# jrkerns/pylinac

Measured on NVIDIA H100. Metric: EPID frames/sec (1024x1024) through PicketFence.analyze(), higher is better.
Workload: dtype u16 pixels / int exact sums / f64 profiles

## Files before the change

pylinac_b200/csrc/common.cuh:

```cuda
#pragma once
#include <cuda_runtime.h>
#include <cstdint>
#include <cstdio>
#include <cstring>
#include <string>
#include <unordered_map>
#include <vector>

#include "../../include/epid.h"

namespace epid {

void set_error(const char* fmt, ...);

#define EPID_CUDA(call)                                                                      \
    do {                                                                                     \
        cudaError_t _e = (call);                                                             \
        if (_e != cudaSuccess) {                                                             \
            ::epid::set_error("%s failed: %s (%s:%d)", #call, cudaGetErrorString(_e), __FILE__, __LINE__); \
            return EPID_ERR_CUDA;                                                            \
        }                                                                                    \
    } while (0)

#define EPID_REQUIRE(cond, code, ...)              \
// ... 19 lines not shown
struct epid_ctx {
    int device = 0;
    int sm_count = 0;
    int cc_major = 0, cc_minor = 0;
    size_t hbm_bytes = 0;
    cudaStream_t stream = nullptr;
    cudaStream_t copy_stream[2] = {nullptr, nullptr};
    int64_t launches = 0;
    void* nccl_comm = nullptr;
    int nranks = 1, rank = 0;
    void* scratch = nullptr;
    size_t scratch_bytes = 0;
    void* scratch2 = nullptr;
    size_t scratch2_bytes = 0;
    void* hist_scratch = nullptr;
    size_t hist_bytes = 0;
    void* inv_scratch = nullptr;
    size_t inv_bytes = 0;
    int stats_exact = 0;
    int64_t stats_uncertified = 0;
    void* pinned = nullptr;
    size_t pinned_bytes = 0;
    void* pinned_ring = nullptr;
    size_t pinned_ring_bytes = 0;
    int pf_exact_only = 0;
    int pf_win2 = 1;
    int64_t pf_fallbacks = 0;
    int64_t pf_redone_frames = 0;
    int64_t pf_exact_frames = 0;
    cudaStream_t redo_stream = nullptr;
    cudaEvent_t ev_front = nullptr, ev_main_done = nullptr, ev_redo_done = nullptr;
    int* h_flags = nullptr;
    std::unordered_map<const void*, size_t> smem_optin;
};

constexpr size_t EPID_BATCH_PAD = 256;
struct epid_batch {
    epid_ctx* ctx = nullptr;
    int dtype = EPID_U16;
    int n = 0, h = 0, w = 0;
    void* dptr = nullptr;
    void* base = nullptr;
    bool owns = true;
    size_t bytes() const { return (size_t)n * h * w * epid::dtype_size(dtype); }
};

namespace epid {
int ensure_scratch(epid_ctx* ctx, size_t bytes);
int ensure_pinned(epid_ctx* ctx, size_t bytes);

template <class K>
inline int smem_opt_in(epid_ctx* ctx, K* kernel, size_t bytes) {
    size_t& cur = ctx->smem_optin[(const void*)kernel];
    if (bytes > cur) {
        EPID_CUDA(cudaFuncSetAttribute(kernel, cudaFuncAttributeMaxDynamicSharedMemorySize, (int)bytes));
        cur = bytes;
    }
    return EPID_OK;
}
#define EPID_SMEM_OPT_IN(ctx, kernel, bytes) do { int _rc = ::epid::smem_opt_in(ctx, kernel, bytes); if (_rc != EPID_OK) return _rc; } while (0)

#ifdef __CUDACC__
__device__ __forceinline__ uint4 ldg_stream16(const void* p) {
    uint4 r;
    asm volatile("ld.global.nc.L1::no_allocate.v4.u32 {%0,%1,%2,%3}, [%4];"
                 : "=r"(r.x), "=r"(r.y), "=r"(r.z), "=r"(r.w)
                 : "l"(p));
    return r;
}

template <typename T>
__device__ __forceinline__ T warp_sum(T v) {
#pragma unroll
    for (int o = 16; o > 0; o >>= 1) v += __shfl_xor_sync(0xffffffffu, v, o);
    return v;
}
template <typename T>
__device__ __forceinline__ T warp_min(T v) {
#pragma unroll
    for (int o = 16; o > 0; o >>= 1) v = min(v, __shfl_xor_sync(0xffffffffu, v, o));
    return v;
}
template <typename T>
__device__ __forceinline__ T warp_max(T v) {
#pragma unroll
    for (int o = 16; o > 0; o >>= 1) v = max(v, __shfl_xor_sync(0xffffffffu, v, o));
    return v;
}
#endif

}
```

pylinac_b200/csrc/pf.cu:

```cuda
#include <cmath>
#include <condition_variable>
#include <cstdlib>
#include <mutex>
#include <thread>
#include <pthread.h>
#include <sched.h>

#define EPID_PK_MAXBLK 2
#include "pf_common.cuh"

namespace epid {

__global__ void k_pf_init(const uint16_t* base, int n, int H0, int W0, int crop, FrameRef* refs, PfFrame* fr, int* counters, const int* __restrict__ sel) {
    const int i = blockIdx.x * blockDim.x + threadIdx.x;
    if (i == 0) { counters[0] = 0; counters[1] = 0; counters[2] = 0; }
    if (i >= n) return;
    refs[i].origin = base + (size_t)(sel ? sel[i] : i) * H0 * W0 + (size_t)crop * W0 + crop;
    refs[i].pitch = W0;
    refs[i].pad = 0;
    PfFrame& f = fr[i];
    f.status = EPID_PF_OK;
    f.noisy = 0;
    f.inv = 0;
    f.corner_inverted = 0;
// ... 83 lines not shown
                            csum[k] += cl;
                            rs += cl;
                        }
                    }
                    rs = warp_sum(rs);
                    if (lane == 0) atomicAdd(&rowsum_sm[rr], rs);
                }
            }
        }
#pragma unroll
        for (int k = 0; k < 8; k++) colpart[tid * 8 + k] = active ? csum[k] : 0u;
        __syncthreads();
        for (int x = tid; x < g.W; x += STATS_THREADS) {
            const int ac = x + mis;
            uint32_t s = 0;
            for (int gg = 0; gg < g.groups; gg++) s += colpart[(gg * g.vprp) * 8 + ac];
            colsum2[(size_t)fi * g.W + x] = s;
        }
        for (int y = tid; y < g.H; y += STATS_THREADS) rowsum2[(size_t)fi * g.H + y] = rowsum_sm[y];
        __syncthreads();
    }
}

__global__ void __launch_bounds__(PROF_THREADS)
k_pf_profile(const PfConst* __restrict__ cc, PfFrame* fr, const uint32_t* __restrict__ rowsum, const uint32_t* __restrict__ colsum,
             const uint32_t* __restrict__ rowsum2, const uint32_t* __restrict__ colsum2) {
    extern __shared__ __align__(16) unsigned char smraw[];
    const int fi = blockIdx.x;
    const PfConst& c = *cc;
    pf_profile_block(c, fr[fi], rowsum + (size_t)fi * c.H, colsum + (size_t)fi * c.W, rowsum2 + (size_t)fi * c.H,
                     colsum2 + (size_t)fi * c.W, smraw);
}

__global__ void __launch_bounds__(WIN_WARPS * 32)
k_pf_windows(const PfConst* __restrict__ cc, const FrameRef* __restrict__ frames, PfFrame* fr, PfWin* __restrict__ wins, int todo_only) {
    __shared__ __align__(16) uint16_t s_px[WIN_WARPS][WIN_CAP_PX];
    __shared__ uint32_t s_m2[WIN_WARPS][WIN_MAX_NC];
    const int fi = blockIdx.y;
    const PfConst& c = *cc;
    PfFrame& f = fr[fi];
    if (f.status != EPID_PF_OK) return;
    if (todo_only && !f.todo) return;
    const int wid = threadIdx.x >> 5, lane = threadIdx.x & 31;
    for (int li = blockIdx.x; li < f.n_inview; li += gridDim.x) {
    const int H = c.H, W = c.W;
    const int orient = f.orientation;
    const int leaf = f.inview[li];
    const double dpmm = c.p.dpmm;
    const double lw_px = c.p.leaf_width_mm[leaf] * dpmm;
    const double lc_px = c.p.leaf_center_mm[leaf] * dpmm + (orient == 0 ? (double)H / 2.0 : (double)W / 2.0);
    const FrameRef frf = frames[fi];
    const int inv = f.inv;
    const uint32_t mn = f.mn, mx = f.mx;
    const double Dd = (double)f.D;
    uint16_t* px = s_px[wid];
    uint32_t* m2 = s_m2[wid];
    double* xs = reinterpret_cast<double*>(px);

    for (int pk = wid; pk < f.n_pickets; pk += WIN_WARPS) {
        PfWin& out = wins[((size_t)fi * PF_L + li) * PF_P + pk];
        if (todo_only && out.valid != -1) continue;
        const double pidx = (double)f.picket_idx[pk];
        const double spacing = f.spacing;
        int a0 = max((int)(pidx - spacing / 2.0), 0);
        int a1 = min((int)(pidx + spacing / 2.0), orient == 0 ? W : H);
        int b0 = max((int)(lc_px - lw_px / 2.0), 0);
        int b1 = min((int)(lc_px + lw_px / 2.0), orient == 0 ? H : W);
        const int nc = a1 - a0, nr = b1 - b0;
        if (nc <= 0 || nr <= 0) {
            if (lane == 0) { out.valid = 0; out.l = 0; out.r = 0; f.status = EPID_PF_WINDOW_NO_PEAK; }
            continue;
        }
        if (nc > WIN_MAX_NC || nr > WIN_MAX_NR) {
            if (lane == 0) { out.valid = 0; f.status = EPID_PF_CAPACITY; }
            continue;
        }
        const int cw = min(nc, WIN_CAP_PX / nr);
        const int sag = c.p.sag_px;
        const int k1 = (nr - 1) / 2, k2 = nr / 2;
        uint32_t gmax = 0;
        unsigned long long rs1[2] = {0, 0}, rs2[2] = {0, 0};
        uint32_t lmin = 0xffffffffu, lmax = 0;
        for (int j0 = 0; j0 < nc; j0 += cw) {
            const int cn = min(cw, nc - j0);
            __syncwarp();
            if (orient == 0) {
                for (int t = lane; t < nr * cn; t += 32) {
                    const int i = t / cn, jj = t - i * cn;
                    int row = b0 + i - sag;
                    row %= H; if (row < 0) row += H;
                    const uint32_t v = __ldg(frf.origin + (size_t)row * frf.pitch + a0 + j0 + jj);
                    const uint32_t g = inv ? mx - v : v - mn;
                    px[i * cn + jj] = (uint16_t)g;
                    gmax = max(gmax, g);
// ... 114 lines not shown
            }
        }
#pragma unroll
        for (int o = 16; o > 0; o >>= 1) {
            const double op = __shfl_xor_sync(0xffffffffu, best_prom, o);
            const int oi = __shfl_xor_sync(0xffffffffu, best_idx, o);
            const int olb = __shfl_xor_sync(0xffffffffu, best_lb, o);
            const int orb = __shfl_xor_sync(0xffffffffu, best_rb, o);
            if (op > best_prom || (op == best_prom && oi > best_idx)) { best_prom = op; best_idx = oi; best_lb = olb; best_rb = orb; }
        }
        if (best_idx < 0) {
            if (lane == 0) { out.valid = 0; f.status = EPID_PF_WINDOW_NO_PEAK; }
            __syncwarp();
            continue;
        }
        if (lane == 0) {
            const int p = best_idx;
            const double h = xs[p] - best_prom * 0.5;
            int k = p;
            while (best_lb < k && h < xs[k]) k--;
            double l = (double)k;
            if (xs[k] < h) l += (h - xs[k]) / (xs[k + 1] - xs[k]);
            k = p;
            while (k < best_rb && h < xs[k]) k++;
            double r = (double)k;
            if (xs[k] < h) r -= (h - xs[k]) / (xs[k - 1] - xs[k]);
            out.valid = 1;
            out.l = l;
            out.r = r;
        }
        __syncwarp();
    }
    }
}

struct PfWork {
    FrameRef* refs;
    FrameRef* refs_b;
    ValueMap* maps;
    PfFrame* fr;
    FrameStats* stats;
    uint32_t *rowsum, *colsum, *rowsum2, *colsum2;
    PfWin* wins;
    epid_pf_summary* summ;
    epid_pf_meas* meas;
    PfConst* cst;
    int* counters;
    int* select;
    int* sel_idx;
    void* front;
    PfWinRec* winrec;
    size_t total;
};

static size_t align_up(size_t v, size_t a) { return (v + a - 1) / a * a; }

static void carve(PfWork& w, char* base, int n, int H, int W, int meas_cap) {
    size_t o = 0;
    auto take = [&](size_t bytes) { char* p = base ? base + o : nullptr; o = align_up(o + bytes, 256); return p; };
    w.refs = (FrameRef*)take(sizeof(FrameRef) * n);
    w.refs_b = (FrameRef*)take(sizeof(FrameRef) * n);
    w.maps = (ValueMap*)take(sizeof(ValueMap) * n);
    w.fr = (PfFrame*)take(sizeof(PfFrame) * n);
    w.stats = (FrameStats*)take(sizeof(FrameStats) * n);
    w.rowsum = (uint32_t*)take(sizeof(uint32_t) * (size_t)n * H);
    w.colsum = (uint32_t*)take(sizeof(uint32_t) * (size_t)n * W);
// ... 236 lines not shown
        ctx->launches++;
        hc.post_filter = 1;
        EPID_CUDA(cudaMemcpyAsync(w.cst, &hc, sizeof(hc), cudaMemcpyHostToDevice, stream));
        StatsGeom g2 = g;
        g2.box = 0;
        rc = launch_frame_stats(ctx, stream, g2, w.refs, n, w.stats, w.rowsum, w.colsum);
        if (rc != EPID_OK) return rc;
        k_pf_decide<<<nb, tb, 0, stream>>>(w.cst, w.stats, w.fr, n, nullptr, 0, w.counters);
        ctx->launches++;
    }
    if (p->orientation < 0) {
        const size_t smem = sizeof(uint32_t) * (size_t)(STATS_THREADS * 8 + H);
        EPID_SMEM_OPT_IN(ctx, k_pf_clamp_sums, 64 * 1024);
        const int grid = n < ctx->sm_count ? n : ctx->sm_count;
        k_pf_clamp_sums<<<grid, STATS_THREADS, smem, stream>>>(g, w.refs, w.fr, n, w.rowsum2, w.colsum2);
        ctx->launches++;
    }
    {
        const size_t smem = pf_profile_smem_bytes(PROF_THREADS, H, W);
        EPID_SMEM_OPT_IN(ctx, k_pf_profile, smem);
        k_pf_profile<<<n, PROF_THREADS, smem, stream>>>(w.cst, w.fr, w.rowsum, w.colsum, w.rowsum2, w.colsum2);
        ctx->launches++;
    }
    if (tm) { rc = tm->mark(stream, PF_STAGE_EXACT_FRONT); if (rc != EPID_OK) return rc; }
    }
    {
        if (hc.win2) {
            rc = launch_pf_windows2(ctx, stream, w.cst, w.refs, w.fr, w.winrec, w.wins, n, tm);
            if (rc != EPID_OK) return rc;
        }
        rc = launch_pf_windows_fast(ctx, stream, w.cst, w.refs, w.fr, w.wins, n);
        if (rc != EPID_OK) return rc;
        if (tm) { rc = tm->mark(stream, PF_STAGE_WINDOWS); if (rc != EPID_OK) return rc; }
        dim3 grid(p->n_leaves < 8 ? p->n_leaves : 8, n);
        k_pf_windows<<<grid, WIN_WARPS * 32, 0, stream>>>(w.cst, w.refs, w.fr, w.wins, 1);
        ctx->launches++;
        if (tm) { rc = tm->mark(stream, PF_STAGE_WINDOWS_GENERIC); if (rc != EPID_OK) return rc; }
    }
    rc = launch_pf_finalize(ctx, stream, w.cst, w.fr, w.wins, w.summ, w.meas, n, meas_cap);
    if (rc != EPID_OK) return rc;
    if (tm) { rc = tm->mark(stream, PF_STAGE_FINALIZE); if (rc != EPID_OK) return rc; }
    EPID_CUDA(cudaGetLastError());
    return EPID_OK;
}

static int ensure_scratch2(epid_ctx* ctx, size_t bytes) {
    if (ctx->scratch2_bytes >= bytes) return EPID_OK;
    if (ctx->scratch2) { EPID_CUDA(cudaStreamSynchronize(ctx->stream)); EPID_CUDA(cudaFree(ctx->scratch2)); ctx->scratch2 = nullptr; ctx->scratch2_bytes = 0; }
    cudaError_t e = cudaMalloc(&ctx->scratch2, bytes);
    if (e != cudaSuccess) { set_error("cudaMalloc(%zu) failed: %s", bytes, cudaGetErrorString(e)); return EPID_ERR_NOMEM; }
    ctx->scratch2_bytes = bytes;
    return EPID_OK;
}

static bool pf_fast_ok(const epid_ctx* ctx, const epid_pf_params* p, int H0, int W0) {
    const int H = H0 - 2 * p->crop_px, W = W0 - 2 * p->crop_px;
    return !ctx->pf_exact_only && p->filter_size == 0 && pf_front_supported(H, W, W0);
}


static int pf_redo_deferred(epid_ctx* ctx, cudaStream_t stream, const uint16_t* d_frames, int m, int H0, int W0, const epid_pf_params* p,
                            int meas_cap, PfWork& w, uint16_t** pools, cudaEvent_t after = nullptr) {
    const int H = H0 - 2 * p->crop_px, W = W0 - 2 * p->crop_px;
    const int Wp = (W + 7) / 8 * 8;
    const int chunk = m < PF_REDO_CHUNK ? m : PF_REDO_CHUNK;
    PfWork rw;
    carve(rw, nullptr, chunk, H, W, meas_cap);
    const size_t work_bytes = align_up(rw.total, 256);
// ... 414 lines not shown
```

pylinac_b200/csrc/pf_common.cuh:

```cuda
#pragma once
#include <cmath>

#include "filters.cuh"
#include "peaks.cuh"
#include "stats.cuh"

namespace epid {

constexpr int PF_P = EPID_PF_MAX_PICKETS;
constexpr int PF_L = EPID_PF_MAX_LEAVES;
constexpr int PROF_THREADS = 256;
constexpr int PROF_MAXN = STATS_MAX_DIM;
constexpr int PROF_PEAK_CAP = 512;
constexpr int WIN_WARPS = 4;
constexpr int WIN_CAP_PX = 4096;
constexpr int WIN_MAX_NC = 1024;
constexpr int WIN_MAX_NR = 64;
constexpr int FIN_THREADS = 256;

constexpr int PF_STATUS_DEFERRED = 90;

struct PfConst {
    epid_pf_params p;
    int H, W;
// ... 7 lines not shown
struct PfFrame {
    int status;
    int noisy;
    int inv;
    int corner_inverted;
    int noise_passes;
    uint32_t mn, mx, D;
    uint32_t med2;
    int orientation;
    int n_pickets;
    int n_inview;
    int todo;
    int win2;
    int picket_idx[PF_P];
    double picket_val[PF_P];
    double spacing;
    short inview[PF_L];
};

struct PfWin { int valid; double l, r; };

constexpr int PF_W2_NCW = 64;
constexpr int PF_W2_NRW = 32;
constexpr int PF_W2_WCAP = 1024;
constexpr int PF_W2_POOL = PF_W2_WCAP * PF_W2_NCW;
struct alignas(16) PfWinRec {
    uint32_t hdr;
    uint32_t moff;
    uint32_t pad[2];
    unsigned long long num[PF_W2_NRW];
    uint32_t ext[PF_W2_NRW];
};
static_assert(sizeof(PfWinRec) == 400, "PfWinRec layout");

__device__ inline void pf_decide_frame(const PfConst& c, const FrameStats& s, PfFrame& f, int check_noise, int* counters) {
    f.mn = s.mn;
    f.mx = s.mx;
    f.D = s.mx - s.mn;
    if (f.D == 0) { f.status = EPID_PF_FLAT_IMAGE; f.noisy = 0; return; }
    if (!c.post_filter) {
        if (check_noise) {
            const double near_min = np_lerp((double)s.ostat[0], (double)s.ostat[1], c.lo.gamma);
            const double near_max = np_lerp((double)s.ostat[2], (double)s.ostat[3], c.hi.gamma);
            const double mnv = (double)s.mn, mxv = (double)s.mx;
            const bool max_is_extreme = mxv > near_max * 1.25;
            const bool min_is_extreme = (mnv < near_min * 0.75) && (fabs(mnv - near_min) > 0.1 * (near_max - near_min));
            f.noisy = (max_is_extreme || min_is_extreme) ? 1 : 0;
            if (f.noisy) atomicAdd(&counters[0], 1);
        }
        const double avg = (double)s.corner_sum / (double)(4 * 10 * 10);
        const double mean = (double)s.sum / (double)s.npix;
        f.corner_inverted = avg > mean ? 1 : 0;
    }
    const int inv = (c.post_filter ? 0 : f.corner_inverted) ^ (c.p.invert ? 1 : 0);
    f.inv = inv;
    const uint32_t a = s.ostat[4], b = s.ostat[5];
    f.med2 = inv ? (s.mx - b) + (s.mx - a) : (a - s.mn) + (b - s.mn);
}


struct PfTimers {
    std::vector<cudaEvent_t> ev;
    bool on = false;
    int record(cudaStream_t s) {
        cudaEvent_t e;
        EPID_CUDA(cudaEventCreate(&e));
// ... 280 lines not shown
```

pylinac_b200/csrc/pf_win_common.cuh:

```cuda
#pragma once
#include <utility>

#include "pf_common.cuh"

namespace epid {

__device__ __forceinline__ unsigned long long mad_wide_u32(uint32_t a, uint32_t b, unsigned long long c) {
    unsigned long long d;
    asm("mad.wide.u32 %0, %1, %2, %3;" : "=l"(d) : "r"(a), "r"(b), "l"(c));
    return d;
}

struct NetList {
    int n;
    short a[640], b[640];
};
constexpr NetList batcher_net(int N) {
    NetList L{};
    for (int p = 1; p < N; p <<= 1)
        for (int k = p; k >= 1; k >>= 1)
            for (int j = k % p; j <= N - 1 - k; j += 2 * k)
                for (int i = 0; i < k; i++)
                    if (i <= N - j - k - 1 && (i + j) / (2 * p) == (i + j + k) / (2 * p)) {
                        L.a[L.n] = (short)(i + j);
                        L.b[L.n] = (short)(i + j + k);
                        L.n++;
                    }
    return L;
}
template <int N>
struct BatcherNet {
    static constexpr NetList L = batcher_net(N);
};

template <int A, int B, int N>
__device__ __forceinline__ void cmpswap_u16x2(uint32_t (&r)[N]) {
    const uint32_t a = r[A], b = r[B];
    r[A] = __vminu2(a, b);
    r[B] = __vmaxu2(a, b);
}
template <int N, int... I>
__device__ __forceinline__ void apply_net_u16x2(uint32_t (&r)[N], std::integer_sequence<int, I...>) {
    (cmpswap_u16x2<BatcherNet<N>::L.a[I], BatcherNet<N>::L.b[I], N>(r), ...);
}
template <int N>
__device__ __forceinline__ void sort_net_u16x2(uint32_t (&r)[N]) {
    apply_net_u16x2<N>(r, std::make_integer_sequence<int, BatcherNet<N>::L.n>{});
}

template <int A, int B, int N>
__device__ __forceinline__ void cmpswap_u64(unsigned long long (&r)[N]) {
    const unsigned long long a = r[A], b = r[B];
    r[A] = a < b ? a : b;
    r[B] = a < b ? b : a;
}
template <int N, int... I>
__device__ __forceinline__ void apply_net_u64(unsigned long long (&r)[N], std::integer_sequence<int, I...>) {
    (cmpswap_u64<BatcherNet<N>::L.a[I], BatcherNet<N>::L.b[I], N>(r), ...);
}
template <int A, int B, int N>
__device__ __forceinline__ void cmpswap_f64(double (&r)[N]) {
    const double a = r[A], b = r[B];
    r[A] = fmin(a, b);
    r[B] = fmax(a, b);
}
template <int N, int... I>
__device__ __forceinline__ void apply_net_f64(double (&r)[N], std::integer_sequence<int, I...>) {
    (cmpswap_f64<BatcherNet<N>::L.a[I], BatcherNet<N>::L.b[I], N>(r), ...);
}
template <int N>
__device__ __forceinline__ void sort_net_f64(double (&r)[N]) {
    apply_net_f64<N>(r, std::make_integer_sequence<int, BatcherNet<N>::L.n>{});
}

template <int N>
__device__ __forceinline__ void sort_net_u64(unsigned long long (&r)[N]) {
    apply_net_u64<N>(r, std::make_integer_sequence<int, BatcherNet<N>::L.n>{});
}

template <int N>
__device__ __forceinline__ void pair_median_exact(const uint16_t* __restrict__ px, int S, int t, uint32_t& m_lo, uint32_t& m_hi) {
    uint32_t r[N];
#pragma unroll
    for (int i = 0; i < N; i++) r[i] = *reinterpret_cast<const uint32_t*>(px + i * S + 2 * t);
    sort_net_u16x2<N>(r);
    const uint32_t va = r[(N - 1) / 2], vb = r[N / 2];
    m_lo = (va & 0xffffu) + (vb & 0xffffu);
    m_hi = (va >> 16) + (vb >> 16);
}

template <int NRP>
__device__ __forceinline__ void pair_median_padded(const uint16_t* __restrict__ px, int S, int nr, int t, uint32_t& m_lo, uint32_t& m_hi) {
    uint32_t r[NRP];
#pragma unroll
    for (int i = 0; i < NRP; i++)
        r[i] = i < nr ? *reinterpret_cast<const uint32_t*>(px + i * S + 2 * t) : 0xffffffffu;
    sort_net_u16x2<NRP>(r);
    const int k1 = (nr - 1) / 2, k2 = nr / 2;
    uint32_t va = 0, vb = 0;
#pragma unroll
    for (int i = 0; i < NRP; i++) {
        if (i == k1) va = r[i];
        if (i == k2) vb = r[i];
    }
    m_lo = (va & 0xffffu) + (vb & 0xffffu);
    m_hi = (va >> 16) + (vb >> 16);
}

static __device__ __noinline__ uint2 pair_median_any(const uint16_t* __restrict__ px, int S, int nr, int t) {
    uint32_t m_lo = 0, m_hi = 0;
    switch (nr) {
#define EPID_MED_CASE(N) case N: pair_median_exact<N>(px, S, t, m_lo, m_hi); break;
        EPID_MED_CASE(6) EPID_MED_CASE(7) EPID_MED_CASE(8) EPID_MED_CASE(9) EPID_MED_CASE(10) EPID_MED_CASE(11)
        EPID_MED_CASE(12) EPID_MED_CASE(13) EPID_MED_CASE(14) EPID_MED_CASE(15) EPID_MED_CASE(16) EPID_MED_CASE(17)
        EPID_MED_CASE(18) EPID_MED_CASE(19) EPID_MED_CASE(20) EPID_MED_CASE(21) EPID_MED_CASE(22) EPID_MED_CASE(23)
        EPID_MED_CASE(24) EPID_MED_CASE(25) EPID_MED_CASE(26) EPID_MED_CASE(27) EPID_MED_CASE(28) EPID_MED_CASE(29)
        EPID_MED_CASE(30) EPID_MED_CASE(31) EPID_MED_CASE(32)
#undef EPID_MED_CASE
        default:
            if (nr < 6) pair_median_padded<8>(px, S, nr, t, m_lo, m_hi);
            else if (nr <= 48) pair_median_padded<48>(px, S, nr, t, m_lo, m_hi);
            else pair_median_padded<64>(px, S, nr, t, m_lo, m_hi);
    }
    return make_uint2(m_lo, m_hi);
}

template <int N>
__device__ __forceinline__ void pair_median_ext_exact(const uint16_t* __restrict__ px, int S, int t, bool want_min, uint32_t& m_lo, uint32_t& m_hi,
                                                      uint32_t& ext2) {
    uint32_t r[N];
#pragma unroll
    for (int i = 0; i < N; i++) r[i] = *reinterpret_cast<const uint32_t*>(px + i * S + 2 * t);
    uint32_t e = r[0];
    if (want_min) {
#pragma unroll
        for (int i = 1; i < N; i++) e = __vminu2(e, r[i]);
    } else {
#pragma unroll
        for (int i = 1; i < N; i++) e = __vmaxu2(e, r[i]);
    }
    ext2 = e;
    sort_net_u16x2<N>(r);
    const uint32_t va = r[(N - 1) / 2], vb = r[N / 2];
    m_lo = (va & 0xffffu) + (vb & 0xffffu);
    m_hi = (va >> 16) + (vb >> 16);
}

template <int NRP>
__device__ __forceinline__ void pair_median_ext_padded(const uint16_t* __restrict__ px, int S, int nr, int t, bool want_min, uint32_t& m_lo,
                                                       uint32_t& m_hi, uint32_t& ext2) {
    uint32_t r[NRP];
    uint32_t e = want_min ? 0xffffffffu : 0u;
#pragma unroll
    for (int i = 0; i < NRP; i++) {
        r[i] = 0xffffffffu;
        if (i < nr) {
            r[i] = *reinterpret_cast<const uint32_t*>(px + i * S + 2 * t);
            e = want_min ? __vminu2(e, r[i]) : __vmaxu2(e, r[i]);
        }
    }
    ext2 = e;
    sort_net_u16x2<NRP>(r);
    const int k1 = (nr - 1) / 2, k2 = nr / 2;
    uint32_t va = 0, vb = 0;
#pragma unroll
    for (int i = 0; i < NRP; i++) {
        if (i == k1) va = r[i];
        if (i == k2) vb = r[i];
    }
    m_lo = (va & 0xffffu) + (vb & 0xffffu);
    m_hi = (va >> 16) + (vb >> 16);
}

static __device__ __noinline__ uint3 pair_median_ext_any(const uint16_t* __restrict__ px, int S, int nr, int t, bool want_min) {
    uint32_t m_lo = 0, m_hi = 0, e = 0;
    switch (nr) {
#define EPID_MED_CASE(N) case N: pair_median_ext_exact<N>(px, S, t, want_min, m_lo, m_hi, e); break;
        EPID_MED_CASE(6) EPID_MED_CASE(7) EPID_MED_CASE(8) EPID_MED_CASE(9) EPID_MED_CASE(10) EPID_MED_CASE(11)
        EPID_MED_CASE(12) EPID_MED_CASE(13) EPID_MED_CASE(14) EPID_MED_CASE(15) EPID_MED_CASE(16) EPID_MED_CASE(17)
        EPID_MED_CASE(18) EPID_MED_CASE(19) EPID_MED_CASE(20) EPID_MED_CASE(21) EPID_MED_CASE(22) EPID_MED_CASE(23)
        EPID_MED_CASE(24) EPID_MED_CASE(25) EPID_MED_CASE(26) EPID_MED_CASE(27) EPID_MED_CASE(28) EPID_MED_CASE(29)
        EPID_MED_CASE(30) EPID_MED_CASE(31) EPID_MED_CASE(32)
#undef EPID_MED_CASE
        default:
            if (nr < 6) pair_median_ext_padded<8>(px, S, nr, t, want_min, m_lo, m_hi, e);
            else pair_median_ext_padded<32>(px, S, nr, t, want_min, m_lo, m_hi, e);
    }
    return make_uint3(m_lo, m_hi, e);
}

template <int ST = 1>
__device__ inline int lb_window_fwxm(const uint32_t* __restrict__ mbase, int nc, double& out_l, double& out_r) {
    auto M = [&](int j) { return mbase[j * ST]; };
    uint32_t lmin, lmax, best1 = 0, best2 = 0;
    {
        int start = -1;
        uint32_t prev = M(0);
        lmin = lmax = prev;
        for (int i = 1; i < nc; i++) {
            const uint32_t v = M(i);
            lmin = min(lmin, v);
            lmax = max(lmax, v);
            if (v < prev && start >= 0) {
                const uint32_t key = (prev << 8) | (uint32_t)((start + i - 1) >> 1);
                if (key > best1) { best2 = best1; best1 = key; }
                else if (key > best2) best2 = key;
            }
            start = v > prev ? i : (v < prev ? -1 : start);
            prev = v;
        }
    }
    if (lmax == lmin || best1 == 0) return 0;
    const double den = (double)(lmax - lmin);
    auto xs = [&](int j) { return (double)(M(j) - lmin) / den; };
    double best_prom = -1.0;
    int best_idx = -1, best_lb = 0, best_rb = 0, best_int = -1;
    auto evaluate = [&](uint32_t key) {
        const uint32_t hp = key >> 8;
        const int p = (int)(key & 255u);
        int k = p, lb = p, rb = p;
        uint32_t lm = hp, rm = hp;
// ... 59 lines not shown
```

pylinac_b200/csrc/pf_windows.cu:

```cuda
#include "pf_common.cuh"
#include "pf_win_common.cuh"

namespace epid {

constexpr int W2_WARPS = 16;
constexpr int W2_POOL = 100 * 1024;
constexpr int W2_MAXNC = 256;
constexpr int W2_GRID_X = 12;

template <int NSL>
__device__ __forceinline__ void row_std_stats(const uint16_t* __restrict__ px, int S, int nr, int nc, double Dd, int lane,
                                              double& sd_max, double& sd_med, int t0, int t1) {
    double sd[NSL];
#pragma unroll
    for (int sl = 0; sl < NSL; sl++) {
        sd[sl] = -1.0;
        const int i = sl * 32 + lane;
        if (i < nr) {
            const uint32_t* __restrict__ rowp = reinterpret_cast<const uint32_t*>(px + i * S);
            uint32_t s1 = 0;
            unsigned long long s2 = 0;
#pragma unroll 4
            for (int t = t0; t < t1; t++) {
                const uint32_t w = rowp[t];
// ... 8 lines not shown
    }
    double m = sd[0];
#pragma unroll
    for (int sl = 1; sl < NSL; sl++) m = fmax(m, sd[sl]);
    sd_max = warp_max(m);
    const int k1 = (nr - 1) / 2, k2 = nr / 2;
    int rank[NSL];
#pragma unroll
    for (int sl = 0; sl < NSL; sl++) rank[sl] = 0;
    for (int t = 0; t < nr; t++) {
        double o;
        if (NSL == 1) o = __shfl_sync(0xffffffffu, sd[0], t);
        else o = __shfl_sync(0xffffffffu, (t >> 5) ? sd[NSL - 1] : sd[0], t & 31);
#pragma unroll
        for (int sl = 0; sl < NSL; sl++) {
            const int me = sl * 32 + lane;
            if (o < sd[sl] || (o == sd[sl] && t < me)) rank[sl]++;
        }
    }
    double ca = 0.0, cb = 0.0;
#pragma unroll
    for (int sl = 0; sl < NSL; sl++) {
        const int me = sl * 32 + lane;
        if (me < nr) {
            if (rank[sl] == k1) ca = sd[sl];
            if (rank[sl] == k2) cb = sd[sl];
        }
    }
    const double med_a = warp_sum(ca);
    const double med_b = warp_sum(cb);
    sd_med = (nr & 1) ? med_a : (med_a + med_b) / 2.0;
}

__global__ void __launch_bounds__(W2_WARPS * 32, 2)
k_pf_windows_fast(const PfConst* __restrict__ cc, const FrameRef* __restrict__ frames, PfFrame* fr, PfWin* __restrict__ wins) {
    extern __shared__ __align__(16) unsigned char smraw[];
    __shared__ int s_geo[4];
    const int fi = blockIdx.y;
    const PfConst& c = *cc;
    PfFrame& f = fr[fi];
    if (f.win2) return;
    const int wid = threadIdx.x >> 5, lane = threadIdx.x & 31;
    const int H = c.H, W = c.W;
    const double dpmm = c.p.dpmm;
    if (wid == 0) {
        const int st = f.status;
        double lw = 0.0;
        for (int i = lane; i < f.n_inview; i += 32) lw = fmax(lw, c.p.leaf_width_mm[f.inview[i]] * dpmm);
        lw = warp_max(lw);
        if (lane == 0) {
            const double sp = f.spacing;
            const int nc_max = (sp == sp && sp < 4096.0) ? (int)sp + 2 : 4096;
            const int nr_max = (int)lw + 2;
            const int s_max = ((nc_max + 14) / 8 + 1) * 8 + 2;
            int stage_b = max(nr_max * s_max * 2, nc_max * 8);
            stage_b = (stage_b + 15) & ~15;
            const int slot = stage_b + ((nc_max * 4 + 15) & ~15);
            s_geo[0] = f.win2 ? -1 : st;
            s_geo[1] = slot;
            s_geo[2] = stage_b;
            s_geo[3] = nc_max > W2_MAXNC + 2 ? 0 : min(W2_WARPS, W2_POOL / slot);
        }
    }
    __syncthreads();
    if (s_geo[0] != EPID_PF_OK) return;
    const int np = f.n_pickets;
    const int total = f.n_inview * np;
    const int active = s_geo[3];
    if (active == 0) {
        for (int widx = blockIdx.x * blockDim.x + threadIdx.x; widx < total; widx += gridDim.x * blockDim.x) {
            const int li = widx / np, pk = widx - li * np;
            wins[((size_t)fi * PF_L + li) * PF_P + pk].valid = -1;
        }
        if (threadIdx.x == 0) f.todo = 1;
        return;
    }
    if (wid >= active) return;
    const int cap_px = s_geo[2] >> 1;
    uint16_t* px = reinterpret_cast<uint16_t*>(smraw + (size_t)wid * s_geo[1]);
    uint32_t* m2 = reinterpret_cast<uint32_t*>(smraw + (size_t)wid * s_geo[1] + s_geo[2]);
    double* xs = reinterpret_cast<double*>(px);
    const int orient = f.orientation;
    const FrameRef frf = frames[fi];
    const int inv = f.inv;
    const uint32_t mn = f.mn, mx = f.mx;
    const uint32_t MN2 = mn * 0x00010001u, MX2 = mx * 0x00010001u;
    const double Dd = (double)f.D;
    const double spacing = f.spacing;
    const int sag = c.p.sag_px;
    const bool aligned = (frf.pitch & 7) == 0;
    const int mis = (int)((reinterpret_cast<uintptr_t>(frf.origin) >> 1) & 7);

    for (int widx = blockIdx.x * active + wid; widx < total; widx += gridDim.x * active) {
        const int li = widx / np, pk = widx - li * np;
        const int leaf = f.inview[li];
        const double lw_px = c.p.leaf_width_mm[leaf] * dpmm;
        const double lc_px = c.p.leaf_center_mm[leaf] * dpmm + (orient == 0 ? (double)H / 2.0 : (double)W / 2.0);
        PfWin& out = wins[((size_t)fi * PF_L + li) * PF_P + pk];
        const double pidx = (double)f.picket_idx[pk];
        const int a0 = max((int)(pidx - spacing / 2.0), 0);
        const int a1 = min((int)(pidx + spacing / 2.0), orient == 0 ? W : H);
        const int b0 = max((int)(lc_px - lw_px / 2.0), 0);
        const int b1 = min((int)(lc_px + lw_px / 2.0), orient == 0 ? H : W);
        const int nc = a1 - a0, nr = b1 - b0;
        if (nc <= 0 || nr <= 0) {
            if (lane == 0) { out.valid = 0; out.l = 0; out.r = 0; f.status = EPID_PF_WINDOW_NO_PEAK; }
            continue;
        }
        const bool vec = orient == 0 && aligned;
        int S, off, nvec = 0, cs = a0;
        if (vec) {
            cs = a0 - ((a0 + mis) & 7);
            const int ce = a1 + ((8 - ((a1 + mis) & 7)) & 7);
            nvec = (ce - cs) >> 3;
            off = a0 - cs;
            S = nvec * 8 + 2;
        } else {
            off = 0;
            S = (nc + 1) & ~1;
            if (((S >> 1) & 1) == 0) S += 2;
        }
        if (nc > W2_MAXNC || nr > 64 || nr * S > cap_px || nc * 4 > s_geo[1] - s_geo[2]) {
            if (lane == 0) { out.valid = -1; f.todo = 1; }
            continue;
        }
        __syncwarp();
// ... 61 lines not shown
            }
        } else {
            const int tot = nc * nr;
            const float inv_nr = 1.0f / (float)nr;
            constexpr int U = 4;
            for (int base = 0; base < tot; base += 32 * U) {
                uint32_t v[U];
                int ii[U], jj[U];
#pragma unroll
                for (int u = 0; u < U; u++) {
                    const int idx = base + u * 32 + lane;
                    jj[u] = (int)(((float)idx + 0.5f) * inv_nr);
                    ii[u] = idx - jj[u] * nr;
                    v[u] = 0;
                    if (idx < tot) {
                        int col = b0 + ii[u] - sag;
                        if (sag) { col %= W; if (col < 0) col += W; }
                        v[u] = __ldg(frf.origin + (size_t)(a0 + jj[u]) * frf.pitch + col);
                    }
                }
#pragma unroll
                for (int u = 0; u < U; u++) {
                    const int idx = base + u * 32 + lane;
                    if (idx >= tot) continue;
                    const uint32_t g = inv ? mx - v[u] : v[u] - mn;
                    gmax = max(gmax, g);
                    px[ii[u] * S + jj[u]] = (uint16_t)g;
                }
            }
            for (int i = lane; i < nr; i += 32)
                for (int jj = nc; jj < S; jj++) px[i * S + jj] = 0;
        }
        {
            const int nwidx = widx + gridDim.x * active;
            if (nwidx < total && orient == 0) {
                const int nli = nwidx / np, npk = nwidx - nli * np;
                const int nleaf = f.inview[nli];
                const double nlw = c.p.leaf_width_mm[nleaf] * dpmm;
                const double nlc = c.p.leaf_center_mm[nleaf] * dpmm + (double)H / 2.0;
                const double npidx = (double)f.picket_idx[npk];
                const int na0 = max((int)(npidx - spacing / 2.0), 0), na1 = min((int)(npidx + spacing / 2.0), W);
                const int nb0 = max((int)(nlc - nlw / 2.0), 0), nb1 = min((int)(nlc + nlw / 2.0), H);
                for (int i = lane; i < nb1 - nb0; i += 32) {
                    int row = nb0 + i - sag;
                    if (sag) { row %= H; if (row < 0) row += H; }
                    const uint16_t* ptr = frf.origin + (size_t)row * frf.pitch + na0;
                    asm volatile("prefetch.global.L2 [%0];" ::"l"(ptr));
                    if (na1 - na0 > 56) asm volatile("prefetch.global.L2 [%0];" ::"l"(ptr + 64));
                    if (na1 - na0 > 120) asm volatile("prefetch.global.L2 [%0];" ::"l"(ptr + 128));
                }
            }
        }
        gmax = warp_max(gmax);
        __syncwarp();
        double sd_max, sd_med;
        const int t0 = off >> 1, t1 = (off + nc + 1) >> 1;
        if (nr <= 32) row_std_stats<1>(px, S, nr, nc, Dd, lane, sd_max, sd_med, t0, t1);
        else row_std_stats<2>(px, S, nr, nc, Dd, lane, sd_max, sd_med, t0, t1);
        const bool above = ((double)gmax / Dd) > c.p.height_threshold * f.picket_val[pk];
        const bool not_edge = sd_max < c.p.edge_threshold * sd_med;
        if (!(above && not_edge)) {
            if (lane == 0) { out.valid = 0; out.l = 0; out.r = 0; }
            continue;
        }
        uint32_t lmin = 0xffffffffu, lmax = 0;
        for (int t = t0 + lane; t < t1; t += 32) {
            const uint2 mm = pair_median_any(px, S, nr, t);
// ... 114 lines not shown
            if (lane == 0) { out.valid = 0; f.status = EPID_PF_WINDOW_NO_PEAK; }
            continue;
        }
        {
            const int p = best_idx;
            const double h = xs[p] - best_prom * 0.5;
            int kl = best_lb;
            for (int c0 = p; c0 > best_lb; c0 -= 32) {
                const int k = c0 - lane;
                const bool stop = k > best_lb && !(h < xs[k]);
                const unsigned b = __ballot_sync(0xffffffffu, stop);
                if (b) { kl = c0 - (__ffs(b) - 1); break; }
            }
            double l = (double)kl;
            if (xs[kl] < h) l += (h - xs[kl]) / (xs[kl + 1] - xs[kl]);
            int kr = best_rb;
            for (int c0 = p; c0 < best_rb; c0 += 32) {
                const int k = c0 + lane;
                const bool stop = k < best_rb && !(h < xs[k]);
                const unsigned b = __ballot_sync(0xffffffffu, stop);
                if (b) { kr = c0 + (__ffs(b) - 1); break; }
            }
            double r = (double)kr;
            if (xs[kr] < h) r -= (h - xs[kr]) / (xs[kr - 1] - xs[kr]);
            if (lane == 0) {
                out.valid = 1;
                out.l = l;
                out.r = r;
            }
        }
    }
}

int launch_pf_windows_fast(epid_ctx* ctx, cudaStream_t stream, const PfConst* cst, const FrameRef* refs, PfFrame* fr, PfWin* wins, int n) {
    const size_t smem = W2_POOL;
    EPID_SMEM_OPT_IN(ctx, k_pf_windows_fast, smem);
    dim3 grid(W2_GRID_X, n);
    k_pf_windows_fast<<<grid, W2_WARPS * 32, smem, stream>>>(cst, refs, fr, wins);
    ctx->launches++;
    EPID_CUDA(cudaGetLastError());
    return EPID_OK;
}

}
```

pylinac_b200/csrc/pf_windows2.cu:

```cuda
#include <cstdio>

#include "pf_common.cuh"
#include "pf_win_common.cuh"
#include "tma.cuh"

namespace epid {

constexpr int WA_WARPS = 8;
constexpr int WA_SLOT = 4416;
constexpr int WA_GRID_X = 4;
constexpr int WA_GMAX = 4;
constexpr int WA_KMAX = 4;
constexpr int WB_THREADS = 128;
constexpr int WB_ST = 33;

__device__ __forceinline__ int wa_row_stride_bytes(int nvec) { return (nvec | 1) * 16; }

struct W2Geo {
    int ok, ntasks;
    int nvmax[WA_GMAX + 1];
    int gtot[WA_GMAX + 1];
};

template <int N>
// ... 225 lines not shown
                        uint32_t e = 0x0000ffffu;
                        if (win_on) {
                            const uint32_t* wp = reinterpret_cast<const uint32_t*>(band + (size_t)r * RS);
                            uint32_t s1 = 0, sA = 0, sB = 0, mx2 = 0, mn2 = 0xffffffffu;
                            auto acc = [&](uint32_t x) {
                                s1 = __dp2a_lo(x, 0x0101u, s1);
                                sA = __dp2a_lo(x, __byte_perm(x, 0u, 0x4431), sA);
                                sB = __dp2a_lo(x, __byte_perm(x, 0u, 0x4420), sB);
                                mx2 = __vmaxu2(mx2, x);
                            };
                            const uint32_t xf = wp[wlo];
                            acc(xf & mfirst);
                            mn2 = __vminu2(mn2, xf | ~mfirst);
#pragma unroll 8
                            for (int w = wlo + 1; w < whi; w++) { const uint32_t x = wp[w]; acc(x); mn2 = __vminu2(mn2, x); }
                            if (whi > wlo) { const uint32_t xl = wp[whi]; acc(xl & mlast); mn2 = __vminu2(mn2, xl | ~mlast); }
                            const unsigned long long s2 = ((unsigned long long)sA << 8) + (unsigned long long)sB;
                            numv = ncl * s2 - (unsigned long long)s1 * s1;
                            e = (max(mx2 & 0xffffu, mx2 >> 16) << 16) | min(mn2 & 0xffffu, mn2 >> 16);
                        }
                        lrec[q].num[r] = numv;
                        lrec[q].ext[r] = e;
                    }
                }
            }
        }
        band_medians(reinterpret_cast<const uint16_t*>(band), RS >> 1, nr, t_lo + lane, t_hi, reinterpret_cast<uint2*>(pool + boff) - t_lo, inv, k2);
        __syncwarp();
    }
}

template <int N, class F>
__device__ __forceinline__ void rank_keys(F key, int nr, unsigned long long& kmax, unsigned long long& ka, unsigned long long& kb) {
    unsigned long long r[N];
    kmax = 0;
#pragma unroll
    for (int i = 0; i < N; i++) {
        r[i] = i < nr ? key(i) : ~0ull;
        if (i < nr && r[i] > kmax) kmax = r[i];
    }
    sort_net_u64<N>(r);
    const int k1 = (nr - 1) / 2, k2 = nr / 2;
    ka = 0; kb = 0;
#pragma unroll
    for (int i = 0; i < N; i++) {
        if (i == k1) ka = r[i];
        if (i == k2) kb = r[i];
    }
}

__global__ void __launch_bounds__(WB_THREADS, 4)
k_pf_win_fwxm(const PfConst* __restrict__ cc, PfFrame* fr, const PfWinRec* __restrict__ recs, const uint32_t* __restrict__ pools,
              PfWin* __restrict__ wins) {
    __shared__ uint32_t s_buf[WB_THREADS / 32][PF_W2_NCW * WB_ST];
    const int fi = blockIdx.y;
    PfFrame& f = fr[fi];
    if (!f.win2) return;
    const PfConst& c = *cc;
    const int np = f.n_pickets;
    const int total = f.n_inview * np;
    const int wid = threadIdx.x >> 5, lane = threadIdx.x & 31;
    const int wbase = blockIdx.x * WB_THREADS + wid * 32;
    if (wbase >= total) return;
    const PfWinRec* frecs = recs + (size_t)fi * PF_W2_WCAP;
    const uint32_t* pool = pools + (size_t)fi * PF_W2_POOL;
    uint32_t* buf = s_buf[wid];
    const int w = wbase + lane;
    const bool active = w < total;
    const PfWinRec& rec = frecs[active ? w : total - 1];
    const uint2 h2 = *reinterpret_cast<const uint2*>(&rec);
    const int my_nc = (int)(short)(h2.x & 0xffffu), my_nr = (int)(short)(h2.x >> 16);
    const uint32_t my_moff = h2.y;
    int li = 0, pk = 0;
    if (active) { li = w / np; pk = w - li * np; }
    PfWin& out = wins[((size_t)fi * PF_L + li) * PF_P + pk];
    bool run = false;
    if (active) {
        if (my_nc <= 0 || my_nr <= 0) {
            out.valid = 0; out.l = 0; out.r = 0; f.status = EPID_PF_WINDOW_NO_PEAK;
        } else {
            run = true;
// ... 77 lines not shown
```

Baseline: 442,200.

## Use persistent occupancy-sized grids with warp-ballot work skipping and pruned selection networks

The fast and generic window kernels now launch a grid sized to resident occupancy instead of one block per frame-part. Each block walks flattened (frame, part) items and uses a warp ballot to skip frames whose gate fails, so idle blocks are no longer launched for filtered-out frames. rank_keys pads with zeros and max values so the medians land at fixed positions, then runs a Batcher network pruned at compile time to only the comparators that affect those two outputs. Unused median/extremum helpers are removed. The trade-off is less parallelism per launch when many frames are active, plus an added __syncthreads per item.

Result: faster. 457,300 (median of 6 runs) (+3.4%).

```diff
diff --git a/pylinac_b200/csrc/common.cuh b/pylinac_b200/csrc/common.cuh
--- a/pylinac_b200/csrc/common.cuh
+++ b/pylinac_b200/csrc/common.cuh
@@ -75,6 +75,7 @@
     cudaEvent_t ev_front = nullptr, ev_main_done = nullptr, ev_redo_done = nullptr;
     int* h_flags = nullptr;
     std::unordered_map<const void*, size_t> smem_optin;
+    std::unordered_map<const void*, int> ctas_per_sm;
 };
 
 constexpr size_t EPID_BATCH_PAD = 256;
@@ -102,6 +103,18 @@
     return EPID_OK;
 }
 #define EPID_SMEM_OPT_IN(ctx, kernel, bytes) do { int _rc = ::epid::smem_opt_in(ctx, kernel, bytes); if (_rc != EPID_OK) return _rc; } while (0)
+
+template <class K>
+inline int resident_grid(epid_ctx* ctx, K* kernel, int threads, size_t smem, long long items, int* grid) {
+    int& per_sm = ctx->ctas_per_sm[(const void*)kernel];
+    if (per_sm == 0) {
+        EPID_CUDA(cudaOccupancyMaxActiveBlocksPerMultiprocessor(&per_sm, kernel, threads, smem));
+        if (per_sm < 1) per_sm = 1;
+    }
+    const long long cap = (long long)per_sm * ctx->sm_count;
+    *grid = (int)(items < cap ? (items > 0 ? items : 1) : cap);
+    return EPID_OK;
+}
 
 #ifdef __CUDACC__
 __device__ __forceinline__ uint4 ldg_stream16(const void* p) {
diff --git a/pylinac_b200/csrc/pf.cu b/pylinac_b200/csrc/pf.cu
--- a/pylinac_b200/csrc/pf.cu
+++ b/pylinac_b200/csrc/pf.cu
@@ -139,17 +139,11 @@
                      colsum2 + (size_t)fi * c.W, smraw);
 }
 
-__global__ void __launch_bounds__(WIN_WARPS * 32)
-k_pf_windows(const PfConst* __restrict__ cc, const FrameRef* __restrict__ frames, PfFrame* fr, PfWin* __restrict__ wins, int todo_only) {
-    __shared__ __align__(16) uint16_t s_px[WIN_WARPS][WIN_CAP_PX];
-    __shared__ uint32_t s_m2[WIN_WARPS][WIN_MAX_NC];
-    const int fi = blockIdx.y;
-    const PfConst& c = *cc;
-    PfFrame& f = fr[fi];
+__device__ __forceinline__ void windows_generic_part(const PfConst& c, const FrameRef* __restrict__ frames, PfFrame& f, PfWin* __restrict__ wins,
+                                                     int fi, int part, int nparts, uint16_t (*s_px)[WIN_CAP_PX], uint32_t (*s_m2)[WIN_MAX_NC]) {
     if (f.status != EPID_PF_OK) return;
-    if (todo_only && !f.todo) return;
     const int wid = threadIdx.x >> 5, lane = threadIdx.x & 31;
-    for (int li = blockIdx.x; li < f.n_inview; li += gridDim.x) {
+    for (int li = part; li < f.n_inview; li += nparts) {
     const int H = c.H, W = c.W;
     const int orient = f.orientation;
     const int leaf = f.inview[li];
@@ -166,7 +160,7 @@
 
     for (int pk = wid; pk < f.n_pickets; pk += WIN_WARPS) {
         PfWin& out = wins[((size_t)fi * PF_L + li) * PF_P + pk];
-        if (todo_only && out.valid != -1) continue;
+        if (out.valid != -1) continue;
         const double pidx = (double)f.picket_idx[pk];
         const double spacing = f.spacing;
         int a0 = max((int)(pidx - spacing / 2.0), 0);
@@ -347,6 +341,14 @@
         __syncwarp();
     }
     }
+}
+
+__global__ void __launch_bounds__(WIN_WARPS * 32)
+k_pf_windows(const PfConst* __restrict__ cc, const FrameRef* __restrict__ frames, PfFrame* fr, PfWin* __restrict__ wins, int n, int nparts) {
+    __shared__ __align__(16) uint16_t s_px[WIN_WARPS][WIN_CAP_PX];
+    __shared__ uint32_t s_m2[WIN_WARPS][WIN_MAX_NC];
+    pf_walk_items(blockIdx.x, gridDim.x, n * nparts, [&](int it) { return fr[it / nparts].todo != 0; },
+                  [&](int it) { windows_generic_part(*cc, frames, fr[it / nparts], wins, it / nparts, it % nparts, nparts, s_px, s_m2); });
 }
 
 struct PfWork {
@@ -649,8 +651,11 @@
         rc = launch_pf_windows_fast(ctx, stream, w.cst, w.refs, w.fr, w.wins, n);
         if (rc != EPID_OK) return rc;
         if (tm) { rc = tm->mark(stream, PF_STAGE_WINDOWS); if (rc != EPID_OK) return rc; }
-        dim3 grid(p->n_leaves < 8 ? p->n_leaves : 8, n);
-        k_pf_windows<<<grid, WIN_WARPS * 32, 0, stream>>>(w.cst, w.refs, w.fr, w.wins, 1);
+        const int nparts = p->n_leaves < 8 ? p->n_leaves : 8;
+        int grid = 0;
+        rc = resident_grid(ctx, k_pf_windows, WIN_WARPS * 32, 0, (long long)n * nparts, &grid);
+        if (rc != EPID_OK) return rc;
+        k_pf_windows<<<grid, WIN_WARPS * 32, 0, stream>>>(w.cst, w.refs, w.fr, w.wins, n, nparts);
         ctx->launches++;
         if (tm) { rc = tm->mark(stream, PF_STAGE_WINDOWS_GENERIC); if (rc != EPID_OK) return rc; }
     }
diff --git a/pylinac_b200/csrc/pf_common.cuh b/pylinac_b200/csrc/pf_common.cuh
--- a/pylinac_b200/csrc/pf_common.cuh
+++ b/pylinac_b200/csrc/pf_common.cuh
@@ -63,6 +63,15 @@
     uint32_t ext[PF_W2_NRW];
 };
 static_assert(sizeof(PfWinRec) == 400, "PfWinRec layout");
+
+template <class Gate, class Body>
+__device__ __forceinline__ void pf_walk_items(int first, int stride, int nitems, Gate gate, Body body) {
+    const int lane = threadIdx.x & 31;
+    for (int base = first; base < nitems; base += 32 * stride) {
+        const int it = base + lane * stride;
+        for (uint32_t m = __ballot_sync(0xffffffffu, it < nitems && gate(it)); m; m &= m - 1) body(base + (__ffs(m) - 1) * stride);
+    }
+}
 
 __device__ inline void pf_decide_frame(const PfConst& c, const FrameStats& s, PfFrame& f, int check_noise, int* counters) {
     f.mn = s.mn;
diff --git a/pylinac_b200/csrc/pf_win_common.cuh b/pylinac_b200/csrc/pf_win_common.cuh
--- a/pylinac_b200/csrc/pf_win_common.cuh
+++ b/pylinac_b200/csrc/pf_win_common.cuh
@@ -11,9 +11,11 @@
     return d;
 }
 
+enum : signed char { NET_BOTH = 0, NET_MIN = 1, NET_MAX = 2 };
 struct NetList {
     int n;
     short a[640], b[640];
+    signed char k[640];
 };
 constexpr NetList batcher_net(int N) {
     NetList L{};
@@ -24,58 +26,67 @@
                     if (i <= N - j - k - 1 && (i + j) / (2 * p) == (i + j + k) / (2 * p)) {
                         L.a[L.n] = (short)(i + j);
                         L.b[L.n] = (short)(i + j + k);
+                        L.k[L.n] = NET_BOTH;
                         L.n++;
                     }
     return L;
+}
+constexpr NetList prune_net(const NetList& L, unsigned long long live) {
+    signed char kind[640] = {};
+    for (int i = L.n - 1; i >= 0; i--) {
+        const unsigned long long ma = 1ull << L.a[i], mb = 1ull << L.b[i];
+        const bool la = (live & ma) != 0, lb = (live & mb) != 0;
+        kind[i] = la && lb ? NET_BOTH : (la ? NET_MIN : (lb ? NET_MAX : (signed char)-1));
+        if (la || lb) live |= ma | mb;
+    }
+    NetList P{};
+    for (int i = 0; i < L.n; i++)
+        if (kind[i] >= 0) {
+            P.a[P.n] = L.a[i];
+            P.b[P.n] = L.b[i];
+            P.k[P.n] = kind[i];
+            P.n++;
+        }
+    return P;
+}
+template <int N, int O1, int O2>
+struct SelectNet {
+    static constexpr NetList L = prune_net(batcher_net(N), (1ull << O1) | (1ull << O2));
+};
+
+template <int A, int B, int K, int N>
+__device__ __forceinline__ void cmpswap_u16x2(uint32_t (&r)[N]) {
+    const uint32_t a = r[A], b = r[B];
+    if constexpr (K != NET_MAX) r[A] = __vminu2(a, b);
+    if constexpr (K != NET_MIN) r[B] = __vmaxu2(a, b);
+}
+template <class Net, int N, int... I>
+__device__ __forceinline__ void apply_net_u16x2(uint32_t (&r)[N], std::integer_sequence<int, I...>) {
+    (cmpswap_u16x2<Net::L.a[I], Net::L.b[I], Net::L.k[I], N>(r), ...);
 }
 template <int N>
 struct BatcherNet {
     static constexpr NetList L = batcher_net(N);
 };
-
-template <int A, int B, int N>
-__device__ __forceinline__ void cmpswap_u16x2(uint32_t (&r)[N]) {
-    const uint32_t a = r[A], b = r[B];
-    r[A] = __vminu2(a, b);
-    r[B] = __vmaxu2(a, b);
-}
-template <int N, int... I>
-__device__ __forceinline__ void apply_net_u16x2(uint32_t (&r)[N], std::integer_sequence<int, I...>) {
-    (cmpswap_u16x2<BatcherNet<N>::L.a[I], BatcherNet<N>::L.b[I], N>(r), ...);
-}
 template <int N>
 __device__ __forceinline__ void sort_net_u16x2(uint32_t (&r)[N]) {
-    apply_net_u16x2<N>(r, std::make_integer_sequence<int, BatcherNet<N>::L.n>{});
-}
-
-template <int A, int B, int N>
+    apply_net_u16x2<BatcherNet<N>>(r, std::make_integer_sequence<int, BatcherNet<N>::L.n>{});
+}
+
+template <int A, int B, int K, int N>
 __device__ __forceinline__ void cmpswap_u64(unsigned long long (&r)[N]) {
     const unsigned long long a = r[A], b = r[B];
-    r[A] = a < b ? a : b;
-    r[B] = a < b ? b : a;
-}
-template <int N, int... I>
+    if constexpr (K != NET_MAX) r[A] = a < b ? a : b;
+    if constexpr (K != NET_MIN) r[B] = a < b ? b : a;
+}
+template <class Net, int N, int... I>
 __device__ __forceinline__ void apply_net_u64(unsigned long long (&r)[N], std::integer_sequence<int, I...>) {
-    (cmpswap_u64<BatcherNet<N>::L.a[I], BatcherNet<N>::L.b[I], N>(r), ...);
-}
-template <int A, int B, int N>
-__device__ __forceinline__ void cmpswap_f64(double (&r)[N]) {
-    const double a = r[A], b = r[B];
-    r[A] = fmin(a, b);
-    r[B] = fmax(a, b);
-}
-template <int N, int... I>
-__device__ __forceinline__ void apply_net_f64(double (&r)[N], std::integer_sequence<int, I...>) {
-    (cmpswap_f64<BatcherNet<N>::L.a[I], BatcherNet<N>::L.b[I], N>(r), ...);
-}
-template <int N>
-__device__ __forceinline__ void sort_net_f64(double (&r)[N]) {
-    apply_net_f64<N>(r, std::make_integer_sequence<int, BatcherNet<N>::L.n>{});
-}
-
-template <int N>
-__device__ __forceinline__ void sort_net_u64(unsigned long long (&r)[N]) {
-    apply_net_u64<N>(r, std::make_integer_sequence<int, BatcherNet<N>::L.n>{});
+    (cmpswap_u64<Net::L.a[I], Net::L.b[I], Net::L.k[I], N>(r), ...);
+}
+template <int N, int O1, int O2>
+__device__ __forceinline__ void select_net_u64(unsigned long long (&r)[N]) {
+    using Net = SelectNet<N, O1, O2>;
+    apply_net_u64<Net>(r, std::make_integer_sequence<int, Net::L.n>{});
 }
 
 template <int N>
@@ -123,70 +134,6 @@
             else pair_median_padded<64>(px, S, nr, t, m_lo, m_hi);
     }
     return make_uint2(m_lo, m_hi);
-}
-
-template <int N>
-__device__ __forceinline__ void pair_median_ext_exact(const uint16_t* __restrict__ px, int S, int t, bool want_min, uint32_t& m_lo, uint32_t& m_hi,
-                                                      uint32_t& ext2) {
-    uint32_t r[N];
-#pragma unroll
-    for (int i = 0; i < N; i++) r[i] = *reinterpret_cast<const uint32_t*>(px + i * S + 2 * t);
-    uint32_t e = r[0];
-    if (want_min) {
-#pragma unroll
-        for (int i = 1; i < N; i++) e = __vminu2(e, r[i]);
-    } else {
-#pragma unroll
-        for (int i = 1; i < N; i++) e = __vmaxu2(e, r[i]);
-    }
-    ext2 = e;
-    sort_net_u16x2<N>(r);
-    const uint32_t va = r[(N - 1) / 2], vb = r[N / 2];
-    m_lo = (va & 0xffffu) + (vb & 0xffffu);
-    m_hi = (va >> 16) + (vb >> 16);
-}
-
-template <int NRP>
-__device__ __forceinline__ void pair_median_ext_padded(const uint16_t* __restrict__ px, int S, int nr, int t, bool want_min, uint32_t& m_lo,
-                                                       uint32_t& m_hi, uint32_t& ext2) {
-    uint32_t r[NRP];
-    uint32_t e = want_min ? 0xffffffffu : 0u;
-#pragma unroll
-    for (int i = 0; i < NRP; i++) {
-        r[i] = 0xffffffffu;
-        if (i < nr) {
-            r[i] = *reinterpret_cast<const uint32_t*>(px + i * S + 2 * t);
-            e = want_min ? __vminu2(e, r[i]) : __vmaxu2(e, r[i]);
-        }
-    }
-    ext2 = e;
-    sort_net_u16x2<NRP>(r);
-    const int k1 = (nr - 1) / 2, k2 = nr / 2;
-    uint32_t va = 0, vb = 0;
-#pragma unroll
-    for (int i = 0; i < NRP; i++) {
-        if (i == k1) va = r[i];
-        if (i == k2) vb = r[i];
-    }
-    m_lo = (va & 0xffffu) + (vb & 0xffffu);
-    m_hi = (va >> 16) + (vb >> 16);
-}
-
-static __device__ __noinline__ uint3 pair_median_ext_any(const uint16_t* __restrict__ px, int S, int nr, int t, bool want_min) {
-    uint32_t m_lo = 0, m_hi = 0, e = 0;
-    switch (nr) {
-#define EPID_MED_CASE(N) case N: pair_median_ext_exact<N>(px, S, t, want_min, m_lo, m_hi, e); break;
-        EPID_MED_CASE(6) EPID_MED_CASE(7) EPID_MED_CASE(8) EPID_MED_CASE(9) EPID_MED_CASE(10) EPID_MED_CASE(11)
-        EPID_MED_CASE(12) EPID_MED_CASE(13) EPID_MED_CASE(14) EPID_MED_CASE(15) EPID_MED_CASE(16) EPID_MED_CASE(17)
-        EPID_MED_CASE(18) EPID_MED_CASE(19) EPID_MED_CASE(20) EPID_MED_CASE(21) EPID_MED_CASE(22) EPID_MED_CASE(23)
-        EPID_MED_CASE(24) EPID_MED_CASE(25) EPID_MED_CASE(26) EPID_MED_CASE(27) EPID_MED_CASE(28) EPID_MED_CASE(29)
-        EPID_MED_CASE(30) EPID_MED_CASE(31) EPID_MED_CASE(32)
-#undef EPID_MED_CASE
-        default:
-            if (nr < 6) pair_median_ext_padded<8>(px, S, nr, t, want_min, m_lo, m_hi, e);
-            else pair_median_ext_padded<32>(px, S, nr, t, want_min, m_lo, m_hi, e);
-    }
-    return make_uint3(m_lo, m_hi, e);
 }
 
 template <int ST = 1>
diff --git a/pylinac_b200/csrc/pf_windows.cu b/pylinac_b200/csrc/pf_windows.cu
--- a/pylinac_b200/csrc/pf_windows.cu
+++ b/pylinac_b200/csrc/pf_windows.cu
@@ -64,14 +64,9 @@
     sd_med = (nr & 1) ? med_a : (med_a + med_b) / 2.0;
 }
 
-__global__ void __launch_bounds__(W2_WARPS * 32, 2)
-k_pf_windows_fast(const PfConst* __restrict__ cc, const FrameRef* __restrict__ frames, PfFrame* fr, PfWin* __restrict__ wins) {
-    extern __shared__ __align__(16) unsigned char smraw[];
-    __shared__ int s_geo[4];
-    const int fi = blockIdx.y;
-    const PfConst& c = *cc;
+__device__ __forceinline__ void windows_fast_part(const PfConst& c, const FrameRef* __restrict__ frames, PfFrame* fr, PfWin* __restrict__ wins,
+                                                  int fi, int part, unsigned char* smraw, int* s_geo) {
     PfFrame& f = fr[fi];
-    if (f.win2) return;
     const int wid = threadIdx.x >> 5, lane = threadIdx.x & 31;
     const int H = c.H, W = c.W;
     const double dpmm = c.p.dpmm;
@@ -100,7 +95,7 @@
     const int total = f.n_inview * np;
     const int active = s_geo[3];
     if (active == 0) {
-        for (int widx = blockIdx.x * blockDim.x + threadIdx.x; widx < total; widx += gridDim.x * blockDim.x) {
+        for (int widx = part * blockDim.x + threadIdx.x; widx < total; widx += W2_GRID_X * blockDim.x) {
             const int li = widx / np, pk = widx - li * np;
             wins[((size_t)fi * PF_L + li) * PF_P + pk].valid = -1;
         }
@@ -123,7 +118,7 @@
     const bool aligned = (frf.pitch & 7) == 0;
     const int mis = (int)((reinterpret_cast<uintptr_t>(frf.origin) >> 1) & 7);
 
-    for (int widx = blockIdx.x * active + wid; widx < total; widx += gridDim.x * active) {
+    for (int widx = part * active + wid; widx < total; widx += W2_GRID_X * active) {
         const int li = widx / np, pk = widx - li * np;
         const int leaf = f.inview[li];
         const double lw_px = c.p.leaf_width_mm[leaf] * dpmm;
@@ -251,7 +246,7 @@
                 for (int jj = nc; jj < S; jj++) px[i * S + jj] = 0;
         }
         {
-            const int nwidx = widx + gridDim.x * active;
+            const int nwidx = widx + W2_GRID_X * active;
             if (nwidx < total && orient == 0) {
                 const int nli = nwidx / np, npk = nwidx - nli * np;
                 const int nleaf = f.inview[nli];
@@ -432,11 +427,23 @@
     }
 }
 
+__global__ void __launch_bounds__(W2_WARPS * 32, 2)
+k_pf_windows_fast(const PfConst* __restrict__ cc, const FrameRef* __restrict__ frames, PfFrame* fr, PfWin* __restrict__ wins, int n) {
+    extern __shared__ __align__(16) unsigned char smraw[];
+    __shared__ int s_geo[4];
+    pf_walk_items(blockIdx.x, gridDim.x, n * W2_GRID_X, [&](int it) { return fr[it / W2_GRID_X].win2 == 0; }, [&](int it) {
+        windows_fast_part(*cc, frames, fr, wins, it / W2_GRID_X, it % W2_GRID_X, smraw, s_geo);
+        __syncthreads();
+    });
+}
+
 int launch_pf_windows_fast(epid_ctx* ctx, cudaStream_t stream, const PfConst* cst, const FrameRef* refs, PfFrame* fr, PfWin* wins, int n) {
     const size_t smem = W2_POOL;
     EPID_SMEM_OPT_IN(ctx, k_pf_windows_fast, smem);
-    dim3 grid(W2_GRID_X, n);
-    k_pf_windows_fast<<<grid, W2_WARPS * 32, smem, stream>>>(cst, refs, fr, wins);
+    int grid = 0;
+    int rc = resident_grid(ctx, k_pf_windows_fast, W2_WARPS * 32, smem, (long long)n * W2_GRID_X, &grid);
+    if (rc != EPID_OK) return rc;
+    k_pf_windows_fast<<<grid, W2_WARPS * 32, smem, stream>>>(cst, refs, fr, wins, n);
     ctx->launches++;
     EPID_CUDA(cudaGetLastError());
     return EPID_OK;
diff --git a/pylinac_b200/csrc/pf_windows2.cu b/pylinac_b200/csrc/pf_windows2.cu
--- a/pylinac_b200/csrc/pf_windows2.cu
+++ b/pylinac_b200/csrc/pf_windows2.cu
@@ -281,21 +281,17 @@
 
 template <int N, class F>
 __device__ __forceinline__ void rank_keys(F key, int nr, unsigned long long& kmax, unsigned long long& ka, unsigned long long& kb) {
+    const int zeros_end = nr + (N - nr + 1) / 2;
     unsigned long long r[N];
     kmax = 0;
 #pragma unroll
     for (int i = 0; i < N; i++) {
-        r[i] = i < nr ? key(i) : ~0ull;
-        if (i < nr && r[i] > kmax) kmax = r[i];
-    }
-    sort_net_u64<N>(r);
-    const int k1 = (nr - 1) / 2, k2 = nr / 2;
-    ka = 0; kb = 0;
-#pragma unroll
-    for (int i = 0; i < N; i++) {
-        if (i == k1) ka = r[i];
-        if (i == k2) kb = r[i];
-    }
+        r[i] = i < nr ? key(i) : (i < zeros_end ? 0ull : ~0ull);
+        if (i < nr) kmax = max(kmax, r[i]);
+    }
+    select_net_u64<N, N / 2 - 1, N / 2>(r);
+    ka = (nr & 1) ? r[N / 2] : r[N / 2 - 1];
+    kb = r[N / 2];
 }
 
 __global__ void __launch_bounds__(WB_THREADS, 4)
```
